# samson6460/tf2_YOLO

Measured on AMD Instinct MI355X. Metric: images/sec training YOLOv3 416x416 bs=32/GPU, higher is better.
Workload: dtype f32-storage/fp16x2-mfma

## Files before the change

tf2_yolo_amd/csrc/conv.hip:

```cpp
#include "conv_args.hpp"
#include <cstdlib>
#include <type_traits>

namespace yolo {

template <int BM, int BN, int WGM, int WGN, bool FLAT>
__global__ __launch_bounds__(256) void gather_conv_kernel(const GatherConvArgs a) {
  constexpr int BK = 32;
  constexpr int LD = BK + 4;
  constexpr int TM = BM / WGM / 32;
  constexpr int TN = BN / WGN / 32;
  constexpr int AR = BM / 32;
  constexpr int BR = BN / 32;
  static_assert(WGM * WGN == 4, "4 waves per block");
  static_assert(TM >= 1 && TN >= 1, "wave tile");

  extern __shared__ __attribute__((aligned(16))) float smem[];
  constexpr int BUF = (BM + BN) * LD;

  const int tid = threadIdx.x;
  const int lane = tid & 63;
  const int wave = tid >> 6;
  const int wm = wave / WGN, wn = wave % WGN;

// ... 974 lines not shown
  YOLO_REQUIRE((C % 16) == 0, "split_planes_concat: the concatenated channel count must be a multiple of 16");
  return launch_split_planes_concat(srcs_host, channels_host, bounds_host, nsrc, rows, planes, dst32, out_bound,
                                    as_stream(stream));
}

extern "C" int yolo_split_planes_concat_ex(const float* const* srcs_host, const int* channels_host,
                                           const float* const* bounds_host, const int* bound_words_host,
                                           const int* upsample_host, int H, int W, int nsrc, long long rows, void* planes,
                                           float* dst32, float* out_bound, void* stream) {
  YOLO_REQUIRE(srcs_host && channels_host && bounds_host && planes && nsrc >= 1 && nsrc <= 4 && rows > 0,
               "split_planes_concat: 1..4 sources, non-null tables");
  int C = 0;
  bool any_up = false;
  for (int i = 0; i < nsrc; ++i) {
    YOLO_REQUIRE(srcs_host[i] && bounds_host[i] && channels_host[i] > 0 && (channels_host[i] % 8) == 0,
                 "split_planes_concat: every source needs a pointer, a bound and a channel count that is a multiple of 8");
    YOLO_REQUIRE(bound_words_host == nullptr || (bound_words_host[i] >= 1 && bound_words_host[i] <= YOLO_INFER_BOUND_WORDS),
                 "split_planes_concat: a bound is 1..%d words", YOLO_INFER_BOUND_WORDS);
    any_up = any_up || (upsample_host != nullptr && upsample_host[i] != 0);
    C += channels_host[i];
  }
  YOLO_REQUIRE((C % 16) == 0, "split_planes_concat: the concatenated channel count must be a multiple of 16");
  YOLO_REQUIRE(!any_up || (H > 0 && W > 0 && (H % 2) == 0 && (W % 2) == 0 && rows % ((long long)H * W) == 0),
               "split_planes_concat: an upsampled source needs even H, W with rows = N * H * W (H=%d W=%d rows=%lld)", H, W, rows);
  return launch_split_planes_concat(srcs_host, channels_host, bounds_host, nsrc, rows, planes, dst32, out_bound,
                                    as_stream(stream), bound_words_host, upsample_host, H, W);
}

extern "C" int yolo_conv2d_fwd_head_unit(const yolo_conv_desc* d, const void* x_planes, const void* w_planes,
                                         const float* bias, int A, int C, int version, const float* anchors, float* t,
                                         float* y, void* stream) {
  return yolo_conv2d_fwd_head_unit_ex(d, x_planes, w_planes, bias, A, C, version, anchors, t, y, YOLO_PREC_F32, stream);
}

extern "C" int yolo_conv2d_fwd_head_unit_ex(const yolo_conv_desc* d, const void* x_planes, const void* w_planes,
                                            const float* bias, int A, int C, int version, const float* anchors, float* t,
                                            float* y, int precision, void* stream) {
  if (int rc = validate_desc(d)) return rc;
  YOLO_REQUIRE_PRECISION(precision, "conv_fwd_head_unit");
  YOLO_REQUIRE(x_planes && w_planes && t && y && A > 0 && C > 0, "conv_fwd_head_unit: bad args");
  YOLO_REQUIRE(d->Cout == A * (5 + C), "conv_fwd_head_unit: Cout = %d is not A (5 + C) = %d", d->Cout, A * (5 + C));
  GatherConvArgs a{};
  a.src = reinterpret_cast<const float*>(x_planes);
  a.wgt = reinterpret_cast<const float*>(w_planes);
  a.bias = bias;
  a.dst = t;
  fill_fwd_args(d, a);
  a.one_pass = precision == YOLO_PREC_F16;
  YOLO_REQUIRE(gather_planes_supported(a), "conv_fwd_head_unit: needs Cin %% 16 == 0 and Cout >= 32");
  if ((version == YOLO_HEAD_V3 || version == YOLO_HEAD_V4) && anchors != nullptr) {
    a.head_y = y;
    a.head_anchors = anchors;
    a.head_A = A;
    a.head_C = C;
    if (conv_small_head_supported(a)) {
      int nwg = 0;
      return launch_conv_small(a, as_stream(stream), &nwg);
    }
    a.head_y = nullptr;
  }
  if (int rc = launch_gather_planes(a, as_stream(stream))) return rc;
  return yolo_head_act_fwd(t, (long long)d->N * d->Ho * d->Wo, A, C, version, anchors, y, stream);
}

extern "C" size_t yolo_planes_bytes(long long rows, int C) {
  if (rows <= 0 || C <= 0 || (C % 16) != 0) return 0;
  return (size_t)planes_bytes(rows, C);
}

extern "C" int yolo_split_planes_batch(const void* jobs, int njobs, long long total_blocks, void* stream) {
  YOLO_REQUIRE(jobs, "split_planes_batch: null job table");
  return launch_split_planes_batch(jobs, njobs, total_blocks, as_stream(stream));
}

extern "C" int yolo_filter_transpose_batch(const void* jobs, int njobs, long long total_blocks, void* stream) {
  YOLO_REQUIRE(jobs, "filter_transpose_batch: null job table");
  return launch_filter_transpose_batch(jobs, njobs, total_blocks, as_stream(stream));
}

extern "C" int yolo_split_planes(const float* x, long long rows, int C, void* planes, void* stream) {
  YOLO_REQUIRE(x && planes, "split_planes: null pointer");
  return launch_split_planes(x, rows, C, planes, as_stream(stream));
}

extern "C" int yolo_split_planes_padded(const float* x, long long rows, int C_src, int C, void* planes, void* stream) {
  YOLO_REQUIRE(x && planes, "split_planes_padded: null pointer");
  return launch_split_planes_padded(x, rows, C_src, C, planes, as_stream(stream));
}

struct BnRedArgs {
  const float* y;
  const float* scale;
  const float* shift;
  const float* mean;
  const float* invstd;
  int act;
  float* part;
  int cap;
  unsigned* aux;
  int nslots;
};
static void set_bnred(GatherConvArgs& a, const BnRedArgs* b) {
  if (b == nullptr) return;
  a.bwd_y = b->y; a.bwd_scale = b->scale; a.bwd_shift = b->shift; a.bwd_mean = b->mean; a.bwd_invstd = b->invstd;
  a.bwd_act = b->act; a.bwd_part = b->part; a.bwd_cap = b->cap; a.bwd_aux = b->aux;
}

static int dgrad_impl(const yolo_conv_desc* d, const float* dy, const float* wT, float* dx, int accumulate,
                      void* stream, bool planes, BnRedArgs* bnred = nullptr) {
  if (int rc = validate_desc(d)) return rc;
  YOLO_REQUIRE(dy && wT && dx, "conv_dgrad: null pointer");
  const bool flat = (d->Cout % 32) != 0;
  YOLO_REQUIRE(!flat || (d->kh == 1 && d->kw == 1 && d->sh == 1 && d->sw == 1),
               "conv_dgrad: Cout %% 32 != 0 only supported for 1x1 stride-1 (head) convs");
  static const bool fuse_classes = env_int("YOLO_DGRAD_CLASSES", 1) != 0;
  if (planes && fuse_classes && d->sh * d->sw > 1 && d->sh * d->sw <= 4) {
    GatherConvArgs a{};
    a.src = dy;
    a.wgt = wT;
    a.dst = dx;
    a.N = d->N; a.Hs = d->Ho; a.Ws = d->Wo; a.Cs = d->Cout;
    a.sy = 1; a.sx = 1;
    a.Hd = d->H; a.Wd = d->W; a.Cd = d->Cin;
    a.osy = d->sh; a.osx = d->sw;
    a.Cout = d->Cin;
    a.ldw = d->kh * d->kw * d->Cout;
    a.accumulate = accumulate;
    a.kw = 1;
    int nt = 0, nc = 0;
    bool ok = true;
    for (int py = 0; py < d->sh && ok; ++py)
      for (int px = 0; px < d->sw && ok; ++px) {
        ClassGeom& c = a.cls[nc++];
        c.Hg = (d->H - py + d->sh - 1) / d->sh;
        c.Wg = (d->W - px + d->sw - 1) / d->sw;
        c.M = (long long)d->N * c.Hg * c.Wg;
        c.ooy = py; c.oox = px; c.tap0 = nt; c.ntaps = 0;
        for (int r = 0; r < d->kh; ++r) {
          const int ty = py + d->pad_t - r;
          if (((ty % d->sh) + d->sh) % d->sh != 0) continue;
          for (int s = 0; s < d->kw; ++s) {
            const int tx = px + d->pad_l - s;
            if (((tx % d->sw) + d->sw) % d->sw != 0) continue;
            a.taps[nt++] = Tap{ty / d->sh, tx / d->sw, (r * d->kw + s) * d->Cout};
            ++c.ntaps;
          }
        }
        if (c.ntaps == 0 || c.Hg <= 0 || c.Wg <= 0) ok = false;
      }
    if (ok) {
      a.ncls = nc;
      a.M = a.cls[0].M; a.Hg = a.cls[0].Hg; a.Wg = a.cls[0].Wg; a.ooy = 0; a.oox = 0; a.ntaps = a.cls[0].ntaps;
      YOLO_REQUIRE(gather_planes_supported(a), "conv_dgrad_planes: needs Cout %% 16 == 0 and Cin >= 32");
      set_bnred(a, bnred);
      const int rc = launch_gather_planes(a, as_stream(stream));
      if (bnred != nullptr) bnred->nslots = a.bwd_nslots;
      return rc;
    }
  }
  YOLO_REQUIRE(bnred == nullptr || d->sh * d->sw == 1,
               "conv_dgrad_planes_bnred: a strided data gradient needs its parity classes in one launch");
  for (int py = 0; py < d->sh; ++py) {
    for (int px = 0; px < d->sw; ++px) {
      GatherConvArgs a{};
      a.src = dy;
      a.wgt = wT;
      a.bias = nullptr;
      a.dst = dx;
      a.N = d->N; a.Hs = d->Ho; a.Ws = d->Wo; a.Cs = d->Cout;
      a.Hg = (d->H - py + d->sh - 1) / d->sh;
      a.Wg = (d->W - px + d->sw - 1) / d->sw;
      if (a.Hg <= 0 || a.Wg <= 0) continue;
      a.sy = 1; a.sx = 1;
      a.Hd = d->H; a.Wd = d->W; a.Cd = d->Cin;
      a.osy = d->sh; a.osx = d->sw; a.ooy = py; a.oox = px;
      a.Cout = d->Cin;
      a.ldw = d->kh * d->kw * d->Cout;
      a.accumulate = accumulate;
      a.kw = 1; a.pad_t = 0; a.pad_l = 0;
      a.M = (long long)d->N * a.Hg * a.Wg;
      int nt = 0;
      for (int r = 0; r < d->kh; ++r) {
        const int ty = py + d->pad_t - r;
        if (((ty % d->sh) + d->sh) % d->sh != 0) continue;
        for (int s = 0; s < d->kw; ++s) {
          const int tx = px + d->pad_l - s;
          if (((tx % d->sw) + d->sw) % d->sw != 0) continue;
          a.taps[nt++] = Tap{ty / d->sh, tx / d->sw, (r * d->kw + s) * d->Cout};
        }
      }
      a.ntaps = nt;
      if (nt == 0) {
        if (!accumulate) {
          a.ntaps = 1;
          a.taps[0] = Tap{-(1 << 20), -(1 << 20), 0};
        } else {
          continue;
        }
      }
      if (planes) {
        YOLO_REQUIRE(gather_planes_supported(a), "conv_dgrad_planes: needs Cout %% 16 == 0 and Cin >= 32");
        set_bnred(a, bnred);
        if (int rc = launch_gather_planes(a, as_stream(stream))) return rc;
        if (bnred != nullptr) bnred->nslots = a.bwd_nslots;
      } else if (int rc = dispatch_gather(a, flat, as_stream(stream))) {
        return rc;
      }
    }
  }
  return YOLO_OK;
}

extern "C" int yolo_conv2d_dgrad(const yolo_conv_desc* d, const float* dy, const float* wT, float* dx, int accumulate,
                                 void* stream) {
  return dgrad_impl(d, dy, wT, dx, accumulate, stream, false);
}

extern "C" int yolo_conv2d_dgrad_planes(const yolo_conv_desc* d, const void* dy_planes, const void* wT_planes, float* dx,
                                        int accumulate, void* stream) {
  return dgrad_impl(d, reinterpret_cast<const float*>(dy_planes), reinterpret_cast<const float*>(wT_planes), dx,
                    accumulate, stream, true);
}

extern "C" int yolo_bnred_slots_cap(const yolo_conv_desc* d) {
  if (d == nullptr) return 0;
  const long long px = (long long)d->N * d->H * d->W;
  const long long cap = px / 64 + 2LL * d->N + 64;
  return cap > 0x7fffffffLL ? 0 : (int)cap;
}

extern "C" int yolo_conv2d_dgrad_planes_bnred(const yolo_conv_desc* d, const void* dy_planes, const void* wT_planes, float* dx,
                                              int accumulate, const float* y, const float* scale, const float* shift,
                                              const float* save_mean, const float* save_invstd, int act, float* partials,
                                              int slots_cap, unsigned* bound_aux, int* nslots, void* stream) {
  YOLO_REQUIRE(d && y && scale && shift && save_mean && save_invstd && partials && nslots && slots_cap > 0,
               "conv_dgrad_planes_bnred: bad args");
  YOLO_REQUIRE(d->Cin % 4 == 0, "conv_dgrad_planes_bnred: Cin=%d must be a multiple of 4", d->Cin);
  YOLO_REQUIRE(act >= 0 && act <= 2, "conv_dgrad_planes_bnred: bad activation %d", act);
  BnRedArgs b{y, scale, shift, save_mean, save_invstd, act, partials, slots_cap, bound_aux, 0};
  const int rc = dgrad_impl(d, reinterpret_cast<const float*>(dy_planes), reinterpret_cast<const float*>(wT_planes), dx,
                            accumulate, stream, true, &b);
  *nslots = b.nslots;
  return rc;
}

static void fill_wgrad_args(const yolo_conv_desc* d, WgradArgs& a) {
  a.N = d->N; a.Hs = d->H; a.Ws = d->W; a.Cs = d->Cin;
  a.Hg = d->Ho; a.Wg = d->Wo;
  a.sy = d->sh; a.sx = d->sw;
  a.Cout = d->Cout;
  a.ldw = d->kh * d->kw * d->Cin;
  a.ntaps = d->kh * d->kw;
  a.kw = d->kw; a.pad_t = d->pad_t; a.pad_l = d->pad_l;
  a.M = (long long)d->N * d->Ho * d->Wo;
}

extern "C" int yolo_conv2d_wgrad_planes(const yolo_conv_desc* d, const void* x_planes, const void* dy_planes, float* dw,
                                        void* stream) {
  if (int rc = validate_desc(d)) return rc;
  YOLO_REQUIRE(x_planes && dy_planes && dw, "conv_wgrad_planes: null pointer");
  WgradArgs a{};
  a.src = reinterpret_cast<const float*>(x_planes);
  a.dy = reinterpret_cast<const float*>(dy_planes);
  a.dw = dw;
  fill_wgrad_args(d, a);
  YOLO_REQUIRE(wgrad_planes_supported(a),
               "conv_wgrad_planes: needs Cin %% 16 == 0, Cout %% 16 == 0, Cout >= 32 and kh*kw*Cin >= 64");
  return launch_wgrad_planes(a, as_stream(stream));
}

extern "C" int yolo_conv2d_wgrad(const yolo_conv_desc* d, const float* x, const float* dy, float* dw, float* dbias,
                                 void* stream) {
  if (int rc = validate_desc(d)) return rc;
  YOLO_REQUIRE(x && dy && dw, "conv_wgrad: null pointer");
  WgradArgs a{};
  a.src = x;
  a.dy = dy;
  a.dw = dw;
  fill_wgrad_args(d, a);
  const bool ascalar = (d->Cout % 4) != 0;
  const bool bflat = (d->Cin % 4) != 0;
  int rc;
  hipStream_t st = as_stream(stream);
  if (g_conv_mode == 1 && wgrad_split_supported(a)) rc = launch_wgrad_split(a, st);
  else if (ascalar && bflat) rc = dispatch_wgrad<true, true>(a, st);
  else if (ascalar) rc = dispatch_wgrad<true, false>(a, st);
  else if (bflat) rc = dispatch_wgrad<false, true>(a, st);
  else rc = dispatch_wgrad<false, false>(a, st);
  if (rc) return rc;
  if (dbias != nullptr) return yolo_conv2d_wgrad_bias(dy, a.M, d->Cout, dbias, stream);
  return YOLO_OK;
}

extern "C" int yolo_conv2d_wgrad_bias(const float* dy, long long P, int Cout, float* dbias, void* stream) {
  YOLO_REQUIRE(dy && dbias && P > 0 && Cout > 0, "conv_wgrad_bias: bad args");
  int cw = 32;
  while (cw < Cout && cw < 256) cw <<= 1;
  dim3 block(cw, 256 / cw);
  const int gy = (Cout + cw - 1) / cw;
  long long gx = (P + block.y * 64 - 1) / (block.y * 64);
  if (gx > 1024) gx = 1024;
  if (gx < 1) gx = 1;
  size_t ws_bytes = 0;
  float* part = reinterpret_cast<float*>(wgrad_workspace(&ws_bytes));
  if (part != nullptr) {
    const long long cap = (long long)(WGRAD_WS_COLSUM_BYTES / 4) / ((long long)block.y * Cout);
// ... 20 lines not shown
```

tf2_yolo_amd/csrc/conv_args.hpp:

```cpp
#pragma once
#include "common.hpp"

namespace yolo {

constexpr int MAX_TAPS = 49;

struct Tap {
  int oy, ox, woff;
};

struct ClassGeom {
  long long M;
  int Hg, Wg, ooy, oox, tap0, ntaps;
};

struct GatherConvArgs {
  const float* src;
  const float* wgt;
  const float* bias;
  float* dst;
  double* stats;
  unsigned* absmax;
  long long M;
  int N, Hs, Ws, Cs;
  int Hg, Wg;
  int sy, sx;
  int Hd, Wd, Cd;
  int osy, osx, ooy, oox;
  int Cout, ldw;
  int ntaps, accumulate;
  int kw, pad_t, pad_l;
  int tiles_n;
  int nblocks;
  unsigned src_bytes, wgt_bytes;
  int zero_blk_src, zero_blk_wgt;
  int nt_store;
  int vec_store;
  int kc;
  int dbg;
  int one_pass;
  const float* epi_scale;
  const float* epi_shift;
  const float* epi_res;
  int epi_act;
  unsigned char* out_planes;
  const float* pl_pred;
  const unsigned* pl_in_bound;
  const unsigned* pl_res_bound;
  int pl_in_n, pl_res_n;
  unsigned* pl_out_words;
  float* head_y;
  const float* head_anchors;
  int head_A, head_C;
  int sk_grid;
  int tile_order;
  float* sk_slabs;
  unsigned* sk_tickets;
  int split_parts;
  int ncls;
  ClassGeom cls[4];
  unsigned long long* stamps;
  const float* bwd_y;
  const float* bwd_scale;
  const float* bwd_shift;
  const float* bwd_mean;
  const float* bwd_invstd;
  float* bwd_part;
  unsigned* bwd_aux;
  int bwd_act;
  int bwd_nslots;
  int bwd_cap;
  Tap taps[MAX_TAPS];
};

#define YOLO_BNRED_CHECK(a)                                                                                          \
  if ((a).bwd_y != nullptr && (a).bwd_nslots > (a).bwd_cap) {                                                        \
    set_error("conv_dgrad(bn reduce): %d partial slots needed, room for %d", (a).bwd_nslots, (a).bwd_cap);           \
    return YOLO_ERR_INVALID_ARG;                                                                                     \
  }

__device__ __forceinline__ int xcd_remap(int bid, int nblocks) {
  const int xcd = bid & 7, idx = bid >> 3;
  const int q = nblocks >> 3, r = nblocks & 7;
  const int start = (xcd < r) ? xcd * (q + 1) : r * (q + 1) + (xcd - r) * q;
  return start + idx;
}


struct WgradArgs {
  const float* src;
  const float* dy;
  float* dw;
  long long M;
  int N, Hs, Ws, Cs;
  int Hg, Wg;
  int sy, sx;
  int Cout, ldw;
  int ntaps;
  int kw, pad_t, pad_l;
  int tiles_co, tiles_j;
  int nblocks;
  long long chunk;
  unsigned src_bytes, dy_bytes;
  int zero_blk_src, zero_blk_dy;
  float* slabs;
  int splits;
};

int launch_gather_split(GatherConvArgs& a, hipStream_t st);
bool gather_split_supported(const GatherConvArgs& a);
long long planes_bytes(long long rows, int C);
int launch_split_planes(const float* x, long long rows, int C, void* planes, hipStream_t st);
int launch_split_planes_absmax(const float* x, long long rows, int C, const unsigned* absmax, const float* extra_bound, int extra_n,
                               void* planes, float* out_bound, hipStream_t st);
int launch_split_planes_concat(const float* const* xs, const int* Cs, const float* const* bounds, int nsrc, long long rows,
                               void* planes, float* dst32, float* out_bound, hipStream_t st,
                               const int* bound_words = nullptr, const int* upsample = nullptr, int H = 0, int W = 0);
int launch_split_planes_padded(const float* x, long long rows, int Csrc, int C, void* planes, hipStream_t st);
int launch_split_planes_batch(const void* jobs, int njobs, long long total_blocks, hipStream_t st);
int launch_filter_transpose_batch(const void* jobs, int njobs, long long total_blocks, hipStream_t st);
int launch_gather_planes(GatherConvArgs& a, hipStream_t st);
bool conv_small_supported(const GatherConvArgs& a);
bool conv_small_head_supported(const GatherConvArgs& a);
int launch_conv_small(GatherConvArgs& a, hipStream_t st, int* nwg);
bool gather_planes_supported(const GatherConvArgs& a);
int conv_split_parts(const GatherConvArgs& a, long long nb, int bm, int min_cb, int idle_div);
int launch_split_reduce(GatherConvArgs& a, int bm, hipStream_t st);
float* conv_split_slabs();
int launch_conv_win(GatherConvArgs& a, int variant, hipStream_t st);
bool conv_win_supported(const GatherConvArgs& a);
enum { OPT_CONV_WIN = 0, OPT_STAMPS = 1, OPT_CONV_SK = 2, OPT_DBG = 3, OPT_TILE_ORDER = 4, OPT_CONV_PATCH = 5, OPT_WGRAD_WIN = 6, OPT_NMS_WALK = 7, OPT_EXP = 8, OPT_COUNT = 16 };
int set_conv_workspace(void* p, size_t bytes, hipStream_t st);
extern void* g_dbg_buf;
extern size_t g_dbg_bytes;
extern int g_opt[OPT_COUNT];
void init_options();
void note_conv_launch(const char* family, int a = 0, int b = 0, int c = 0, int d = 0);
int launch_wgrad_planes(WgradArgs& a, hipStream_t st);
bool wgrad_planes_supported(const WgradArgs& a);
int launch_wgrad_win(WgradArgs& a, hipStream_t st);
bool wgrad_win_supported(const WgradArgs& a);
constexpr size_t WGRAD_WS_COLSUM_BYTES = 1 << 20;
void* wgrad_workspace(size_t* bytes);
bool stem_fwd_supported(const yolo_conv_desc* d);
struct StemEpiArgs {
  const float* scale;
  const float* shift;
  int act;
  void* planes;
  const float* pred;
  const unsigned* in_words;
  int in_n;
  unsigned* out_words;
};
bool stem_infer_supported(const yolo_conv_desc* d);
int launch_stem_filter_prep(const float* w, const float* bias, float* wt, hipStream_t st);
int launch_absmax_words(const float* x, long long n, unsigned* words, int* n_words, hipStream_t st);
int launch_stem_infer(const yolo_conv_desc* d, const float* x, const float* wt, float* y, const StemEpiArgs& e, int* out_n,
                      hipStream_t st);
size_t stem_bwd_scratch_bytes();
int launch_stem_bn_bwd_wgrad(const yolo_conv_desc* d, const float* y, const float* dout, const float* img, const float* scale,
                             const float* shift, const float* smean, const float* sinv, int act, const double* redsum,
                             float* dgamma, float* dbeta, float* dw, float* scratch, size_t scratch_bytes, hipStream_t st);
int launch_stem_fwd(const yolo_conv_desc* d, const float* x, const float* w, const float* bias, float* y, double* stats,
                    unsigned* absmax, hipStream_t st);
int launch_wgrad_split(WgradArgs& a, hipStream_t st);
bool wgrad_split_supported(const WgradArgs& a);

}
```

tf2_yolo_amd/csrc/runtime.hip:

```cpp
#include "conv_args.hpp"
#include <cstdlib>
#include <cstring>

namespace yolo {

static thread_local char g_err[512] = "";

void set_error(const char* fmt, ...) {
  va_list ap;
  va_start(ap, fmt);
  vsnprintf(g_err, sizeof(g_err), fmt, ap);
  va_end(ap);
}

static thread_local struct { const char* family; int v[4]; int launches; } g_conv_note = {"", {0, 0, 0, 0}, 0};
static thread_local char g_conv_name[96] = "";

void note_conv_launch(const char* family, int a, int b, int c, int d) {
  g_conv_note = {family, {a, b, c, d}, g_conv_note.launches + 1};
}

int g_opt[OPT_COUNT];
void* g_dbg_buf = nullptr;
size_t g_dbg_bytes = 0;
static void options_from_env() {
  for (int i = 0; i < OPT_COUNT; ++i) g_opt[i] = 0;
  g_opt[OPT_CONV_WIN] = env_int("YOLO_CONV_WIN", 1);
  g_opt[OPT_CONV_SK] = env_int("YOLO_CONV_SK", 1);
  g_opt[OPT_CONV_PATCH] = env_int("YOLO_CONV_PATCH", 1);
  g_opt[OPT_WGRAD_WIN] = env_int("YOLO_WGRAD_WIN", 1);
  g_opt[OPT_NMS_WALK] = env_int("YOLO_NMS_WALK", 0);
  g_opt[OPT_EXP] = env_int("YOLO_EXP", 0);
}
void init_options() {
  static bool done = false;
  if (done) return;
  done = true;
  options_from_env();
}

}

extern "C" int yolo_set_option(int key, int value) {
  yolo::init_options();
  if (key == -1) {
    yolo::options_from_env();
    return YOLO_OK;
  }
  if (key < 0 || key >= yolo::OPT_COUNT) {
    yolo::set_error("yolo_set_option: unknown key %d", key);
    return YOLO_ERR_INVALID_ARG;
  }
  yolo::g_opt[key] = value;
  return YOLO_OK;
}

extern "C" size_t yolo_conv_workspace_bytes(void) { return (size_t)(1 << 20) + (size_t)512 * 2 * 256 * 128 * 4; }

extern "C" int yolo_set_conv_workspace(void* p, size_t bytes, void* stream) {
  yolo::init_options();
  return yolo::set_conv_workspace(p, bytes, yolo::as_stream(stream));
}

extern "C" int yolo_set_debug_buffer(void* p, size_t bytes) {
  yolo::g_dbg_buf = p;
  yolo::g_dbg_bytes = bytes;
  return YOLO_OK;
}

extern "C" const char* yolo_last_error(void) { return yolo::g_err; }

extern "C" const char* yolo_last_conv_kernel(int* launches) {
  auto& n = yolo::g_conv_note;
  snprintf(yolo::g_conv_name, sizeof(yolo::g_conv_name), n.family, n.v[0], n.v[1], n.v[2], n.v[3]);
  if (launches != nullptr) *launches = n.launches;
  n = {"", {0, 0, 0, 0}, 0};
  return yolo::g_conv_name;
}

extern "C" int yolo_abi_version(void) { return 5; }

#include <dlfcn.h>
namespace {
using nccl_allreduce_fn = int (*)(const void*, void*, size_t, int, int, void*, hipStream_t);
nccl_allreduce_fn find_nccl_allreduce() {
  void* f = dlsym(RTLD_DEFAULT, "ncclAllReduce");
  if (f == nullptr) {
    void* h = dlopen("librccl.so.1", RTLD_NOW | RTLD_GLOBAL);
    if (h == nullptr) h = dlopen("librccl.so", RTLD_NOW | RTLD_GLOBAL);
    if (h != nullptr) f = dlsym(h, "ncclAllReduce");
  }
  return reinterpret_cast<nccl_allreduce_fn>(f);
}
}

extern "C" int yolo_allreduce_bucket(void* rccl_comm, float* grads, long long count, void* stream) {
  YOLO_REQUIRE(rccl_comm != nullptr && grads != nullptr && count > 0, "allreduce_bucket: bad args");
  static nccl_allreduce_fn fn = find_nccl_allreduce();
  if (fn == nullptr) {
    yolo::set_error("allreduce_bucket: no RCCL in this process (ncclAllReduce not found, librccl.so not loadable)");
    return YOLO_ERR_LAUNCH;
  }
  constexpr int kNcclFloat = 7, kNcclSum = 0;
  const int rc = fn(grads, grads, (size_t)count, kNcclFloat, kNcclSum, rccl_comm, yolo::as_stream(stream));
  if (rc != 0) {
    yolo::set_error("allreduce_bucket: ncclAllReduce returned %d", rc);
    return YOLO_ERR_LAUNCH;
  }
  return YOLO_OK;
}

extern "C" int yolo_device_available(void) {
  int n = 0;
  if (hipGetDeviceCount(&n) != hipSuccess) return 0;
  return n > 0 ? 1 : 0;
}
```

tf2_yolo_amd/ops.py:

```python
import ctypes
from ctypes import byref, c_void_p

import torch

from . import _lib
from . import tape as _tape
from ._lib import ConvDesc, LossCfg, YoloHipError, check

BN_EPS = 1e-3
BN_MOMENTUM = 0.99
BN_STAT_SLOTS = 64
BN_RED_SLOTS = 512
SPLIT_BATCH_UNITS = 4


class KernelTimer:

    def __init__(self):
        self.pending = []

    def bracket(self, flops, fn, layer=None):
        last, n = _lib.load().yolo_last_conv_kernel, ctypes.c_int(0)
        last(None)
        s, e = torch.cuda.Event(enable_timing=True), torch.cuda.Event(enable_timing=True)
        s.record()
        fn()
        e.record()
        name = last(byref(n)).decode()
        if not name:
            raise YoloHipError("KernelTimer: the bracketed call launched no convolution kernel")
        self.pending.append((name, flops, n.value, s, e, layer))

    def summary(self, by_layer=False):
        torch.cuda.synchronize()
        agg = {}
        for name, flops, launches, s, e, layer in self.pending:
            a = agg.setdefault((name, layer) if by_layer else name, {"launches": 0, "ms": 0.0, "flops": 0.0})
            a["launches"] += launches
            a["ms"] += s.elapsed_time(e)
            a["flops"] += flops
        self.pending = []
        return agg


TIMER = None


def _conv_flops(d):
    return 2.0 * d.N * d.Ho * d.Wo * d.Cout * d.kh * d.kw * d.Cin


def _layer_key(d, which):
    return (which, d.H, d.W, d.Cin, d.Cout, d.kh, d.sh, d.N)


import os as _os
CONV_MODE = "fp32" if _os.environ.get("YOLO_CONV_MODE", "split")[:1] in ("f", "0") else "split"
USE_PLANES = CONV_MODE == "split" and _os.environ.get("YOLO_CONV_PLANES", "1") != "0"


def planes_fwd_ok(cin, cout):
    return USE_PLANES and cin % 16 == 0 and cout >= 32


def planes_dgrad_ok(cin, cout):
    return USE_PLANES and cout % 16 == 0 and cin >= 32


def planes_wgrad_ok(cin, cout, taps, stride=1):
    return USE_PLANES and cin % 16 == 0 and cout % 16 == 0 and cout >= 32 and taps * cin >= 64


OPT_CONV_WIN = 0
OPT_CONV_SK = 2
OPT_CONV_PATCH = 5
OPT_WGRAD_WIN = 6
OPT_NMS_WALK = 7
_CONV_WS = None


def ensure_conv_workspace():
    global _CONV_WS
    if _CONV_WS is not None and _CONV_WS.device.index != torch.cuda.current_device():
        raise YoloHipError(f"libyolo_hip.so was initialised on cuda:{_CONV_WS.device.index} and cannot also serve "
                           f"cuda:{torch.cuda.current_device()}: start one process per GPU")
    if _CONV_WS is None:
        lib = _lib.load()
        n = int(lib.yolo_conv_workspace_bytes())
        _CONV_WS = torch.empty(n, dtype=torch.uint8, device="cuda")
        check(lib.yolo_set_conv_workspace(_p(_CONV_WS), n, _stream()), "yolo_set_conv_workspace")
    return _CONV_WS


_WGRAD_WS = None


def ensure_wgrad_workspace():
    global _WGRAD_WS
    if _WGRAD_WS is None:
        lib = _lib.load()
        n = int(lib.yolo_wgrad_workspace_bytes())
        _WGRAD_WS = torch.empty(n, dtype=torch.uint8, device="cuda")
        check(lib.yolo_set_wgrad_workspace(_p(_WGRAD_WS), n), "yolo_set_wgrad_workspace")
    return _WGRAD_WS


_SIDE_STREAMS = {}


def _overlaps(a, b, cycles=6000000):
    e0, e1, e2 = (torch.cuda.Event(enable_timing=True) for _ in range(3))
    torch.cuda.synchronize()
    with torch.cuda.stream(a):
        e0.record(a)
        torch.cuda._sleep(cycles)
        e1.record(a)
    torch.cuda.synchronize()
    one = e0.elapsed_time(e1)
    with torch.cuda.stream(a):
        e0.record(a)
    b.wait_event(e0)
    with torch.cuda.stream(b):
        torch.cuda._sleep(cycles)
    with torch.cuda.stream(a):
        torch.cuda._sleep(cycles)
    a.wait_stream(b)
    e2.record(a)
    torch.cuda.synchronize()
    return e0.elapsed_time(e2) < 1.5 * one


def _first_use(st, dev):
    with torch.cuda.device(dev):
        torch.zeros(1, device=f"cuda:{dev}")
        with torch.cuda.stream(st):
            torch.zeros(1, device=f"cuda:{dev}")
        torch.cuda.current_stream().wait_stream(st)


def create_side_streams(device=None):
    dev = torch.cuda.current_device() if device is None else torch.device(device).index
    if dev is None:
        dev = torch.cuda.current_device()
    for role in ("wgrad", "comm"):
        if (dev, role) not in _SIDE_STREAMS:
            st = torch.cuda.Stream(device=dev)
            if (_os.environ.get("YOLO_STREAM_PROBE") == "1" and dev == torch.cuda.current_device()
                    and not _overlaps(torch.cuda.current_stream(), st)):
                import warnings
                warnings.warn(f"tf2_yolo_amd: the {role} stream shares a hardware queue with the compute stream: the step "
                              "will run them one after the other (create_side_streams() earlier, or raise GPU_MAX_HW_QUEUES)")
            _SIDE_STREAMS[(dev, role)] = st
            _first_use(st, dev)
    return {role: _SIDE_STREAMS[(dev, role)] for role in ("wgrad", "comm")}


def concurrent_stream(role, beside=None, device=None):
    st = create_side_streams(device)[role]
    want = torch.cuda.current_device() if device is None else torch.device(device).index
    if want is not None and st.device.index != want:
        raise YoloHipError(f"side stream of role {role!r} lives on cuda:{st.device.index}, not on cuda:{want}")
    return st


def set_option(key, value):
    check(_lib.load().yolo_set_option(int(key), int(value)), "yolo_set_option")


def reset_options():
    check(_lib.load().yolo_set_option(-1, 0), "yolo_set_option")


def _stream():
    return c_void_p(torch.cuda.current_stream().cuda_stream)


def _p(t):
    if t is None:
        return c_void_p(0)
    if _tape.ACTIVE is not None:
        _tape.ACTIVE.keep.append(t)
    return c_void_p(t.data_ptr())


def _chk_f32(*ts):
    for t in ts:
        if t is None:
            continue
        if not (t.is_cuda and t.dtype == torch.float32 and t.is_contiguous()):
            raise YoloHipError("expected a contiguous float32 CUDA tensor, got "
                               f"{t.dtype} {t.device} contiguous={t.is_contiguous()}")


def same_pad(size, k, s):
    out = -(-size // s)
    total = max((out - 1) * s + k - size, 0)
    return out, total // 2


def conv_desc(x_shape, cout, kh, kw, stride, padding):
    n, h, w, cin = x_shape
    if padding == "same":
        ho, pt = same_pad(h, kh, stride)
        wo, pl = same_pad(w, kw, stride)
    elif padding == "valid":
        ho, wo, pt, pl = (h - kh) // stride + 1, (w - kw) // stride + 1, 0, 0
    elif padding == "darknet_s2":
        ho, wo, pt, pl = (h + 1 - kh) // stride + 1, (w + 1 - kw) // stride + 1, 1, 1
    else:
        raise ValueError(f"bad padding {padding}")
    return ConvDesc(n, h, w, cin, cout, kh, kw, ho, wo, stride, stride, pt, pl)


def conv2d_fwd(d, x, w, bias=None, out=None, stats=None, absmax=None):
    _chk_f32(x, w, bias)
    if out is None:
        out = torch.empty((d.N, d.Ho, d.Wo, d.Cout), device=x.device, dtype=torch.float32)
    if x.numel() != d.N * d.H * d.W * d.Cin or w.numel() != d.Cout * d.kh * d.kw * d.Cin:
        raise YoloHipError("conv2d_fwd: tensor sizes do not match the descriptor")
    if out.numel() != d.N * d.Ho * d.Wo * d.Cout:
        raise YoloHipError("conv2d_fwd: output size does not match the descriptor")
    if stats is not None and stats.numel() != BN_STAT_SLOTS * 2 * d.Cout:
        raise YoloHipError("conv2d_fwd: stats must hold BN_STAT_SLOTS x 2 x Cout doubles")
    def run():
        check(_lib.load().yolo_conv2d_fwd_absmax(byref(d), _p(x), _p(w), _p(bias), _p(out), _p(stats), _p(absmax),
                                                 _stream()), "yolo_conv2d_fwd")
    if TIMER is not None:
        TIMER.bracket(_conv_flops(d), run)
    else:
# ... 1152 lines not shown
```

Before: 1070.

## Add fused stride-2 3x3 dgrad kernel computing all four parity classes per tile

Adds a dedicated data-gradient kernel for 3x3 stride-2 convolutions. It loads one shared dy window per 16x16 tile into LDS and computes all four output parity classes from that window with fp16 split-plane MFMA. The window and the 9 filter taps are double-buffered through LDS using DMA, and results are staged to scatter interleaved outputs. It runs by default in auto mode only when Cout equals 32 and there are at least 512 workgroups; otherwise it falls back to the generic gather-planes path.

```diff
diff --git a/tf2_yolo_amd/csrc/conv.hip b/tf2_yolo_amd/csrc/conv.hip
--- a/tf2_yolo_amd/csrc/conv.hip
+++ b/tf2_yolo_amd/csrc/conv.hip
@@ -1150,6 +1150,12 @@
       a.ncls = nc;
       a.M = a.cls[0].M; a.Hg = a.cls[0].Hg; a.Wg = a.cls[0].Wg; a.ooy = 0; a.oox = 0; a.ntaps = a.cls[0].ntaps;
       YOLO_REQUIRE(gather_planes_supported(a), "conv_dgrad_planes: needs Cout %% 16 == 0 and Cin >= 32");
+      init_options();
+      if (g_opt[OPT_DGRAD_S2] != 0 && bnred == nullptr && nc == 4 && d->kh == 3 && d->kw == 3 && d->sh == 2 && d->sw == 2 &&
+          d->Cout % 16 == 0 && d->Cin % 32 == 0) {
+        const int rc = launch_dgrad_s2(a, g_opt[OPT_DGRAD_S2], as_stream(stream));
+        if (rc <= 0) return rc;
+      }
       set_bnred(a, bnred);
       const int rc = launch_gather_planes(a, as_stream(stream));
       if (bnred != nullptr) bnred->nslots = a.bwd_nslots;
diff --git a/tf2_yolo_amd/csrc/conv_args.hpp b/tf2_yolo_amd/csrc/conv_args.hpp
--- a/tf2_yolo_amd/csrc/conv_args.hpp
+++ b/tf2_yolo_amd/csrc/conv_args.hpp
@@ -129,7 +129,8 @@
 float* conv_split_slabs();
 int launch_conv_win(GatherConvArgs& a, int variant, hipStream_t st);
 bool conv_win_supported(const GatherConvArgs& a);
-enum { OPT_CONV_WIN = 0, OPT_STAMPS = 1, OPT_CONV_SK = 2, OPT_DBG = 3, OPT_TILE_ORDER = 4, OPT_CONV_PATCH = 5, OPT_WGRAD_WIN = 6, OPT_NMS_WALK = 7, OPT_EXP = 8, OPT_COUNT = 16 };
+int launch_dgrad_s2(GatherConvArgs& a, int mode, hipStream_t st);
+enum { OPT_CONV_WIN = 0, OPT_STAMPS = 1, OPT_CONV_SK = 2, OPT_DBG = 3, OPT_TILE_ORDER = 4, OPT_CONV_PATCH = 5, OPT_WGRAD_WIN = 6, OPT_NMS_WALK = 7, OPT_EXP = 8, OPT_DGRAD_S2 = 9, OPT_COUNT = 16 };
 int set_conv_workspace(void* p, size_t bytes, hipStream_t st);
 extern void* g_dbg_buf;
 extern size_t g_dbg_bytes;
diff --git a/tf2_yolo_amd/csrc/conv_dgrad_s2.hip b/tf2_yolo_amd/csrc/conv_dgrad_s2.hip
--- /dev/null
+++ b/tf2_yolo_amd/csrc/conv_dgrad_s2.hip
@@ -0,0 +1,238 @@
+#include "planes.hpp"
+#include <algorithm>
+
+namespace yolo {
+
+constexpr int DS2_P = 16;
+constexpr int DS2_WW = DS2_P + 1;
+constexpr int DS2_SLOTS = 320;
+constexpr int DS2_UNIT_BYTES = DS2_SLOTS * 16;
+constexpr int DS2_WIN_BYTES = 4 * DS2_UNIT_BYTES;
+constexpr int DS2_NB = 9;
+constexpr int DS2_BN = 32;
+constexpr int DS2_STAGE_BYTES = DS2_WIN_BYTES + DS2_NB * PL_PLANES * 1024;
+constexpr int DS2_LDS_BYTES = 2 * DS2_STAGE_BYTES;
+constexpr int DS2_PITCH = DS2_BN + 4;
+constexpr int DS2_STRIP_FLOATS = 4 * 2 * DS2_P * DS2_PITCH;
+static_assert(DS2_WW * DS2_WW <= DS2_SLOTS && DS2_SLOTS % 64 == 0, "window slots: whole DMA instructions");
+static_assert(4 * DS2_STRIP_FLOATS * 4 <= DS2_LDS_BYTES, "the four waves' output strips reuse the stage buffers");
+
+struct DgradS2Args {
+  const unsigned char* dy;
+  const unsigned char* wt;
+  float* dx;
+  unsigned dy_bytes, wt_bytes;
+  int zero_blk_dy;
+  int N, Hs, Ws, Cs;
+  int Hd, Wd, Cd;
+  int ldw;
+  int oy0, ox0;
+  int tiles_y, tiles_x, tiles_n, nblocks;
+  int accumulate, nt_store;
+  int bslot[4][4];
+  int wrec[DS2_NB];
+};
+
+__global__ __launch_bounds__(256, 2) void conv_dgrad_s2_planes_kernel(const DgradS2Args a) {
+  extern __shared__ __attribute__((aligned(16))) unsigned char smem[];
+  const unsigned lds_base = (unsigned)(size_t)smem;
+  const int tid = threadIdx.x;
+  const int lane = tid & 63;
+  const int wave = __builtin_amdgcn_readfirstlane(tid >> 6);
+
+  const int tile = xcd_remap((int)blockIdx.x, a.nblocks);
+  const int tile_n = tile % a.tiles_n;
+  int patch = tile / a.tiles_n;
+  const int tx = patch % a.tiles_x;
+  patch /= a.tiles_x;
+  const int ty = patch % a.tiles_y;
+  const int img = patch / a.tiles_y;
+  const int y0 = ty * DS2_P, x0 = tx * DS2_P, n0 = tile_n * DS2_BN;
+
+  const unsigned strideA = (unsigned)((a.Cs >> 4) * PL_RECORD);
+  const unsigned strideB = (unsigned)((a.ldw >> 4) * PL_RECORD);
+  const i32x4 rsrcA = planes_rsrc(a.dy, a.dy_bytes), rsrcB = planes_rsrc(a.wt, a.wt_bytes);
+  unsigned wvoff[DS2_SLOTS / 64];
+#pragma unroll
+  for (int j = 0; j < DS2_SLOTS / 64; ++j) {
+    const int slot = j * 64 + lane;
+    const int wy = slot / DS2_WW, wx = slot - wy * DS2_WW;
+    const int ys = y0 + a.oy0 + wy, xs = x0 + a.ox0 + wx;
+    const bool ok = slot < DS2_WW * DS2_WW && (unsigned)ys < (unsigned)a.Hs && (unsigned)xs < (unsigned)a.Ws;
+    const int pix = (img * a.Hs + ys) * a.Ws + xs;
+    wvoff[j] = (ok ? ((unsigned)pix >> 4) : (unsigned)a.zero_blk_dy) * strideA + (ok ? (pix & 15) * 16 : 0) + wave * 256;
+  }
+  const int fr = lane & 31, hf = lane >> 5;
+  const int co = n0 + fr;
+  const unsigned bvoff = (unsigned)(co >> 4) * strideB + (co & 15) * 16 + hf * 256;
+  constexpr int ND_B = DS2_NB * PL_PLANES;
+  auto issue_stage = [&](int cb, int buf) {
+    const unsigned lb = lds_base + buf * DS2_STAGE_BYTES;
+#pragma unroll
+    for (int j = 0; j < DS2_SLOTS / 64; ++j)
+      dma16(rsrcA, wvoff[j], (unsigned)cb * PL_RECORD, __builtin_amdgcn_readfirstlane(lb + wave * DS2_UNIT_BYTES + j * 1024));
+#pragma unroll
+    for (int k = 0; k < (ND_B + 3) / 4; ++k) {
+      const int d = wave + 4 * k;
+      if (d < ND_B) {
+        const unsigned so = __builtin_amdgcn_readfirstlane((unsigned)(a.wrec[d >> 1] + cb) * PL_RECORD + (d & 1) * 512);
+        dma16(rsrcB, bvoff, so, __builtin_amdgcn_readfirstlane(lb + DS2_WIN_BYTES + d * 1024));
+      }
+    }
+  };
+
+  const int Hg0 = (a.Hd + 1) >> 1;
+  bool blk_ok[2];
+  unsigned abase[2];
+#pragma unroll
+  for (int i = 0; i < 2; ++i) {
+    const int prow = (wave * 2 + i) * 2;
+    blk_ok[i] = y0 + prow < Hg0;
+    abase[i] = hf * DS2_UNIT_BYTES + ((prow + (fr >> 4)) * DS2_WW + (fr & 15)) * 16;
+  }
+
+  f32x16 acc[4][2];
+#pragma unroll
+  for (int c = 0; c < 4; ++c)
+#pragma unroll
+    for (int i = 0; i < 2; ++i)
+#pragma unroll
+      for (int q = 0; q < 16; ++q) acc[c][i][q] = 0.f;
+
+  const int ncb = a.Cs >> 4;
+  issue_stage(0, 0);
+  for (int cb = 0; cb < ncb; ++cb) {
+    const int buf = cb & 1;
+    asm volatile("s_waitcnt vmcnt(0) lgkmcnt(0)" ::: "memory");
+    __builtin_amdgcn_s_barrier();
+    if (cb + 1 < ncb) issue_stage(cb + 1, buf ^ 1);
+    const unsigned char* win = smem + buf * DS2_STAGE_BYTES;
+    const unsigned char* fil = win + DS2_WIN_BYTES + lane * 16;
+    if (!blk_ok[0]) continue;
+#pragma unroll
+    for (int s = 0; s < 4; ++s) {
+      f16x8 fa[PL_PLANES][2];
+#pragma unroll
+      for (int p = 0; p < PL_PLANES; ++p)
+#pragma unroll
+        for (int i = 0; i < 2; ++i)
+          fa[p][i] = *reinterpret_cast<const f16x8*>(win + abase[i] + p * 2 * DS2_UNIT_BYTES + ((s >> 1) * DS2_WW + (s & 1)) * 16);
+#pragma unroll
+      for (int c = 0; c < 4; ++c) {
+        const int j = a.bslot[s][c];
+        if (j >= 0) {
+          const f16x8 fbh = *reinterpret_cast<const f16x8*>(fil + (j * PL_PLANES + 0) * 1024);
+          const f16x8 fbl = *reinterpret_cast<const f16x8*>(fil + (j * PL_PLANES + 1) * 1024);
+#pragma unroll
+          for (int q = 0; q < 3; ++q)
+#pragma unroll
+            for (int i = 0; i < 2; ++i)
+              acc[c][i] = __builtin_amdgcn_mfma_f32_32x32x16_f16(fa[q == 0 ? 1 : 0][i], q == 1 ? fbl : fbh, acc[c][i], 0, 0, 0);
+        }
+      }
+    }
+  }
+  asm volatile("s_waitcnt vmcnt(0) lgkmcnt(0)" ::: "memory");
+  __syncthreads();
+
+  const float unscale = reinterpret_cast<const float*>(a.dy + a.dy_bytes - PL_HEADER)[2] *
+                        reinterpret_cast<const float*>(a.wt + a.wt_bytes - PL_HEADER)[2];
+  float* strip = reinterpret_cast<float*>(smem) + wave * DS2_STRIP_FLOATS;
+#pragma unroll
+  for (int i = 0; i < 2; ++i) {
+    if (!blk_ok[i]) continue;
+#pragma unroll
+    for (int c = 0; c < 4; ++c)
+#pragma unroll
+      for (int q = 0; q < 16; ++q) {
+        const int orow = 2 * (q >> 3) + (c >> 1);
+        const int opx = 2 * ((q & 3) + 8 * ((q >> 2) & 1) + 4 * hf) + (c & 1);
+        strip[(orow * 2 * DS2_P + opx) * DS2_PITCH + fr] = acc[c][i][q] * unscale;
+      }
+    asm volatile("s_waitcnt lgkmcnt(0)" ::: "memory");
+    const int oy_base = 2 * (y0 + (wave * 2 + i) * 2), ox_base = 2 * x0;
+#pragma unroll
+    for (int h0 = 0; h0 < 16; h0 += 4) {
+      const int oy = oy_base + (h0 >> 2);
+      f32x4 v[4];
+      float* p[4];
+      bool ok[4];
+#pragma unroll
+      for (int k = 0; k < 4; ++k) {
+        const int opx = k * 8 + (lane >> 3), c4 = lane & 7;
+        const int ox = ox_base + opx;
+        ok[k] = oy < a.Hd && ox < a.Wd;
+        p[k] = a.dx + (((long long)img * a.Hd + oy) * a.Wd + ox) * a.Cd + n0 + c4 * 4;
+        v[k] = *reinterpret_cast<const f32x4*>(strip + ((h0 >> 2) * 2 * DS2_P + opx) * DS2_PITCH + c4 * 4);
+        if (ok[k] && a.accumulate) v[k] += *reinterpret_cast<const f32x4*>(p[k]);
+      }
+#pragma unroll
+      for (int k = 0; k < 4; ++k)
+        if (ok[k]) {
+          if (a.nt_store) __builtin_nontemporal_store(v[k], reinterpret_cast<f32x4*>(p[k]));
+          else *reinterpret_cast<f32x4*>(p[k]) = v[k];
+        }
+    }
+    asm volatile("s_waitcnt lgkmcnt(0)" ::: "memory");
+  }
+}
+
+static bool dgrad_s2_auto(const GatherConvArgs& g, long long workgroups) { return g.Cout == DS2_BN && workgroups >= 512; }
+
+int launch_dgrad_s2(GatherConvArgs& g, int mode, hipStream_t st) {
+  if (g.ncls != 4 || g.osy != 2 || g.osx != 2 || (g.Cs % 16) != 0 || (g.Cout % DS2_BN) != 0 || g.Cd != g.Cout ||
+      g.bwd_y != nullptr || g.bias != nullptr || g.stats != nullptr)
+    return 1;
+  if ((reinterpret_cast<uintptr_t>(g.dst) & 15) != 0) return 1;
+  DgradS2Args a{};
+  int oy0 = 1 << 30, oy1 = -(1 << 30), ox0 = 1 << 30, ox1 = -(1 << 30);
+  for (int c = 0; c < 4; ++c) {
+    const ClassGeom& k = g.cls[c];
+    if (k.ooy != (c >> 1) || k.oox != (c & 1)) return 1;
+    for (int t = k.tap0; t < k.tap0 + k.ntaps; ++t) {
+      oy0 = std::min(oy0, g.taps[t].oy); oy1 = std::max(oy1, g.taps[t].oy);
+      ox0 = std::min(ox0, g.taps[t].ox); ox1 = std::max(ox1, g.taps[t].ox);
+    }
+  }
+  if (oy1 - oy0 > 1 || ox1 - ox0 > 1) return 1;
+  for (int s = 0; s < 4; ++s)
+    for (int c = 0; c < 4; ++c) a.bslot[s][c] = -1;
+  int nact = 0;
+  for (int c = 0; c < 4; ++c) {
+    const ClassGeom& k = g.cls[c];
+    for (int t = k.tap0; t < k.tap0 + k.ntaps; ++t) {
+      const int s = 2 * (g.taps[t].oy - oy0) + (g.taps[t].ox - ox0);
+      if (a.bslot[s][c] >= 0 || nact >= DS2_NB || (g.taps[t].woff % 16) != 0) return 1;
+      a.bslot[s][c] = nact;
+      a.wrec[nact++] = g.taps[t].woff >> 4;
+    }
+  }
+  const long long rowsA = (long long)g.N * g.Hs * g.Ws;
+  const long long bytesA = planes_bytes(rowsA, g.Cs), bytesB = planes_bytes(g.Cout, g.ldw);
+  if (bytesA >= (1LL << 32) || bytesB >= (1LL << 32)) return 1;
+  a.dy = reinterpret_cast<const unsigned char*>(g.src);
+  a.wt = reinterpret_cast<const unsigned char*>(g.wgt);
+  a.dx = g.dst;
+  a.dy_bytes = (unsigned)bytesA; a.wt_bytes = (unsigned)bytesB;
+  a.zero_blk_dy = (int)((rowsA + 15) / 16);
+  a.N = g.N; a.Hs = g.Hs; a.Ws = g.Ws; a.Cs = g.Cs;
+  a.Hd = g.Hd; a.Wd = g.Wd; a.Cd = g.Cd;
+  a.ldw = g.ldw;
+  a.oy0 = oy0; a.ox0 = ox0;
+  a.tiles_y = ((g.Hd + 1) / 2 + DS2_P - 1) / DS2_P;
+  a.tiles_x = ((g.Wd + 1) / 2 + DS2_P - 1) / DS2_P;
+  a.tiles_n = g.Cout / DS2_BN;
+  const long long nb = (long long)g.N * a.tiles_y * a.tiles_x * a.tiles_n;
+  if (nb <= 0 || nb > 0x7fffffffLL) return 1;
+  if (mode == 1 && !dgrad_s2_auto(g, nb)) return 1;
+  a.nblocks = (int)nb;
+  a.accumulate = g.accumulate;
+  static const int nt = env_int("YOLO_NT_STORE", 1);
+  a.nt_store = nt;
+  if (!lds_limit_ok<&conv_dgrad_s2_planes_kernel, DS2_LDS_BYTES>("conv_dgrad_s2_planes_kernel")) return 1;
+  note_conv_launch("conv_dgrad_s2_planes_kernel<%d,%d>", DS2_P * DS2_P, DS2_BN);
+  hipLaunchKernelGGL(conv_dgrad_s2_planes_kernel, dim3((unsigned)nb), dim3(256), DS2_LDS_BYTES, st, a);
+  return check_launch("conv_dgrad_s2_planes_kernel");
+}
+
+}
diff --git a/tf2_yolo_amd/csrc/runtime.hip b/tf2_yolo_amd/csrc/runtime.hip
--- a/tf2_yolo_amd/csrc/runtime.hip
+++ b/tf2_yolo_amd/csrc/runtime.hip
@@ -31,6 +31,7 @@
   g_opt[OPT_WGRAD_WIN] = env_int("YOLO_WGRAD_WIN", 1);
   g_opt[OPT_NMS_WALK] = env_int("YOLO_NMS_WALK", 0);
   g_opt[OPT_EXP] = env_int("YOLO_EXP", 0);
+  g_opt[OPT_DGRAD_S2] = env_int("YOLO_DGRAD_S2", 1);
 }
 void init_options() {
   static bool done = false;
diff --git a/tf2_yolo_amd/ops.py b/tf2_yolo_amd/ops.py
--- a/tf2_yolo_amd/ops.py
+++ b/tf2_yolo_amd/ops.py
@@ -75,6 +75,7 @@
 OPT_CONV_SK = 2
 OPT_CONV_PATCH = 5
 OPT_WGRAD_WIN = 6
+OPT_DGRAD_S2 = 9
 OPT_NMS_WALK = 7
 _CONV_WS = None
 
```

Result: no change. 1077 (median of 6 runs) (+0.7%).
